# google/forma

Hardware: AMD Instinct MI355X
Metric: frames/sec (sorted+painted, device-resident) + Mpixel-segments/sec (higher is better)
Workload: dtype u64 segments / f64+f32 rasterizer / f32 painter; 1 GPU; paris-like-30k-4k (labelled stand-in: paris-30k.svg is not in the reference checkout); layers=30000, pixel_segments=13757174, frames_in_flight=3

## Files before the change

forma_amd/_lib.py:

```python
from __future__ import annotations

import ctypes as C
import os
import subprocess

_HERE = os.path.dirname(os.path.abspath(__file__))
CSRC = os.path.join(_HERE, "csrc")
SO_PATH = os.environ.get("FORMA_HIP_LIB") or os.path.join(CSRC, "libforma_hip.so")

NONE = 0xFFFFFFFF

ERRORS = {0: "FORMA_OK", -1: "FORMA_E_ARG", -2: "FORMA_E_HIP", -3: "FORMA_E_NO_DEVICE", -4: "FORMA_E_CAPACITY",
          -5: "FORMA_E_STATE", -6: "FORMA_E_INTERNAL", -7: "FORMA_E_COMM"}


class FormaError(RuntimeError):
    def __init__(self, code, msg=""):
        self.code = code
        super().__init__(f"{ERRORS.get(code, code)}: {msg}")


class GeomT(C.Structure):
    _fields_ = [("order", C.c_uint32), ("flags", C.c_uint32), ("xf", C.c_float * 6)]

# ... 18 lines not shown

class ContextInfoT(C.Structure):
    _fields_ = [("n_devices", C.c_uint32), ("frames_in_flight", C.c_uint32), ("transport", C.c_uint32), ("layout", C.c_uint32),
                ("devices", C.c_int32 * 8)]


class KernelTimeT(C.Structure):
    _fields_ = [("name", C.c_char * 48), ("start_us", C.c_float), ("us", C.c_float), ("stage", C.c_uint32), ("reserved", C.c_uint32)]


class SortPlanT(C.Structure):
    _fields_ = [("n_passes", C.c_uint32), ("biased", C.c_uint32), ("shift", C.c_uint32 * 12), ("mask", C.c_uint32 * 12), ("bias", C.c_uint32 * 12)]


class FlattenTablesT(C.Structure):
    _fields_ = [("point_commands", C.c_void_p), ("point_indices", C.c_void_p), ("quad_indices", C.c_void_p), ("n_points", C.c_size_t),
                ("qx", C.c_void_p), ("qy", C.c_void_p), ("qw", C.c_void_p), ("x0", C.c_void_p), ("dx_recip", C.c_void_p),
                ("k0", C.c_void_p), ("dk", C.c_void_p), ("curvatures_recip", C.c_void_p), ("partial_spline", C.c_void_p),
                ("partial_curv", C.c_void_p), ("n_quads", C.c_size_t), ("sp0x", C.c_void_p), ("sp0y", C.c_void_p),
                ("sp2x", C.c_void_p), ("sp2y", C.c_void_p), ("n_splines", C.c_size_t)]


class AffineRangeT(C.Structure):
    _fields_ = [("first", C.c_uint64), ("count", C.c_uint64), ("m", C.c_float * 6)]


class KeepRangeT(C.Structure):
    _fields_ = [("first", C.c_uint64), ("count", C.c_uint64)]


class CountersT(C.Structure):
    _fields_ = [("geometry_points", C.c_uint64), ("geometry_uploads", C.c_uint64), ("geometry_appends", C.c_uint64),
                ("geometry_retains", C.c_uint64), ("geometry_bytes_h2d", C.c_uint64), ("geometry_bytes_d2h", C.c_uint64),
                ("frames", C.c_uint64), ("frames_learned", C.c_uint64), ("frames_rerun", C.c_uint64)]

    def as_dict(self):
        return {k: int(getattr(self, k)) for k, _ in self._fields_}


_vp, _sz, _u32, _i = C.c_void_p, C.c_size_t, C.c_uint32, C.c_int
SYMBOLS = {
    "forma_hip_create": (_i, [C.POINTER(_vp), _i]),
    "forma_hip_create_multi": (_i, [C.POINTER(_vp), C.POINTER(_i), _i]),
    "forma_hip_destroy": (None, [_vp]),
    "forma_hip_last_error": (C.c_char_p, [_vp]),
    "forma_hip_version": (C.c_char_p, []),
    "forma_hip_set_geometry": (_i, [_vp, _vp, _vp, _vp, _sz]),
    "forma_hip_set_geoms": (_i, [_vp, _vp, _sz]),
    "forma_hip_set_styles": (_i, [_vp, _vp, _sz, _vp, _sz, _vp]),
    "forma_hip_set_images": (_i, [_vp, _vp, _sz, _vp, _sz]),
    "forma_hip_flatten": (_i, [_vp, _vp, _vp, _vp]),
    "forma_hip_geometry_append": (_i, [_vp, _vp, _vp, _vp, _sz]),
    "forma_hip_geometry_retain": (_i, [_vp, _vp, _sz, _vp, _sz]),
    "forma_hip_read_geometry": (_i, [_vp, _vp, _vp, _vp, _sz, _vp]),
    "forma_hip_counters": (_i, [_vp, _vp]),
    "forma_hip_prepare_lines": (_i, [_vp, _u32, _u32] + [_vp] * 10),
    "forma_hip_rasterize": (_i, [_vp, _sz] + [_vp] * 10 + [_vp, _sz, _vp]),
    "forma_hip_sort": (_i, [_vp, _vp, _sz, _i]),
    "forma_hip_paint": (_i, [_vp, _vp, _sz, _vp, _u32, _u32, _sz, _vp, _vp, _vp]),
    "forma_hip_render": (_i, [_vp, _vp, _u32, _u32, _sz, _vp, _vp, _vp, _i, _vp]),
    "forma_hip_render_enqueue": (_i, [_vp, _vp, _u32, _u32, _sz, _vp, _vp, _vp]),
    "forma_hip_render_device": (_i, [_vp, _vp, _u32, _u32, _u32, _sz, _vp, _vp, _vp, _i, _vp, _vp]),
    "forma_hip_register_buffer": (_i, [_vp, _vp, _sz]),
    "forma_hip_unregister_buffer": (_i, [_vp, _vp]),
    "forma_hip_cache_clear": (_i, [_vp, _i]),
    "forma_hip_set_frames_in_flight": (_i, [_vp, _i]),
    "forma_hip_multi_layout": (_i, [_vp, _i]),
# ... 48 lines not shown
```

forma_amd/csrc/api.cpp:

```cpp
#include <new>

#include "ctx.h"

#ifndef FORMA_ARCH
#define FORMA_ARCH "gfx950"
#endif

thread_local KernelTimer* g_ktimer = nullptr;
static inline float* kt_us(forma_hip_ctx* c) { return c->kt_dur_us; }

int fd_fail(forma_hip_ctx* c, int code, const char* what, hipError_t e) {
    if (c) snprintf(c->err, sizeof c->err, "%s%s%s", what, e != hipSuccess ? ": " : "", e != hipSuccess ? hipGetErrorString(e) : "");
    return code;
}

namespace {

inline int fail(forma_hip_ctx* c, int code, const char* what, hipError_t e = hipSuccess) { return fd_fail(c, code, what, e); }
void share_scene(forma_hip_ctx* o);
void invalidate_counts(forma_hip_ctx* o);
inline forma_hip_ctx* last_slot(forma_hip_ctx* ctx) { return ctx->last ? ctx->last : ctx; }
#define HIPCHECK(expr)                                                        \
    do {                                                                      \
        hipError_t _e = (expr);                                               \
// ... 102 lines not shown
    ctx->n_lines = n_lines;
    ctx->n_seg = 0; ctx->n_compact = 0; ctx->have_unsorted = true; ctx->live44 = 0; ctx->layer_sorted = true;
    ctx->speculated = false; ctx->ras_hist_on = false; ctx->ras_fused = false;
    ctx->pz = forma_hip_ctx::PreZero();
    int rc = reset_info(ctx);
    if (rc) return rc;
    if (n_lines == 0) return FORMA_OK;
    const LineSource S = geometry_source(ctx, width, height);
    if ((rc = run_line_table(ctx, S, n_lines, timing, bound_n, zero))) return rc;
    if (zero && cleared) ctx->pz = *cleared;
    FrameInfo* dinfo = ctx->info.as<FrameInfo>();
    DevCount nc_seg, nc_cmp;
    if (bound_n) {
        nc_seg = DevCount{&dinfo->n_segments, bound_n};
        nc_cmp = DevCount{&dinfo->n_compact, (uint32_t)n_lines};
    } else {
        const size_t N = ctx->n_seg;
        if (N == 0) return FORMA_OK;
        if (N >= (1ull << 30)) return fail(ctx, FORMA_E_CAPACITY, "more than 2^30-1 pixel segments on one device");
        nc_seg = DevCount{nullptr, (uint32_t)N};
        nc_cmp = DevCount{nullptr, (uint32_t)ctx->n_compact};
    }
    HIPCHECK(ctx->seg_u.ensure(((size_t)nc_seg.bound + SEG_PAD) * 8));
    HIPCHECK(ctx->ras_masks.ensure(((size_t)nc_seg.bound / RAS_TILE + 2) * 32));
    RasHist RH;
    memset(&RH, 0, sizeof RH);
    if (hist_too && bound_n && ctx->pred_valid && ctx->pz.sort_p && ctx->pz.sort_p == ctx->sort_counters.p && !ctx->dbg.no_ras_hist) {
        ctx->ras_plan = frame_sort_plan(ctx, ctx->pred_live44, ctx->pred_layer_sorted, ctx->digit_bits, true, nullptr);
        RH = make_ras_hist(ctx->ras_plan, ctx->sort_counters.as<uint32_t>());
        ctx->ras_hist_on = RH.hist != nullptr;
        if (RH.hist && ctx->pz.slice_p && ctx->pz.slice_p == ctx->slice_buf.p && ctx->pz.slice_words >= slice_tab_words(bound_n) &&
            fuse_plan_ok(ctx, ctx->ras_plan)) {
            const SliceSrc SS = make_slice_src(ctx->slice_buf.as<uint32_t>(), bound_n);
            RH.slice_tab = SS.tab; RH.tab_stride = SS.tab_stride;
            ctx->ras_fused = true;
        }
        {
            const SortPlan plain = make_segment_sort_plan(ctx->pred_live44, ctx->pred_layer_sorted, ctx->digit_bits, nullptr, nullptr);
            const SortPlan lay = ctx->pred_layer_sorted ? SortPlan{} : make_sort_plan((ctx->pred_live44 & 0x1FFFFFull) << 20, 20, 41, ctx->digit_bits);
            bool biased = false;
            for (int p = 0; p < ctx->ras_plan.n_passes; p++) biased |= ctx->ras_plan.fmask[p] != 0u;
            RH.track_range = (biased || plain.n_passes > (ctx->pred_layer_sorted ? 0 : lay.n_passes) + 2) ? 1u : 0u;
        }
    }
    stage_begin(ctx, ST_RASTER, timing);
    launch_rasterize(ctx->stream, S, nc_cmp, nc_seg, ctx->cl_idx.as<uint32_t>(), ctx->cl_start.as<uint32_t>(),
                     ctx->block_first.as<uint32_t>(), ctx->seg_u.as<uint64_t>(), dinfo, (int)ctx->band_row0,
                     (int)ctx->band_row1, ctx->ras_masks.as<uint32_t>(), bound_n == 0, &RH);
    ctx->pending_masks = bound_n ? PendingMasks{ctx->ras_masks.as<uint32_t>(), 0u, ctx->ras_hist_on ? 1u : 0u} : PendingMasks{nullptr, 0u, 0u};
    ctx->seg_u_fused = ctx->ras_fused; ctx->fused_w = width; ctx->fused_h = height;
    stage_end(ctx, ST_RASTER, timing);
    HIPCHECK(hipGetLastError());
    ctx->speculated = (speculate || bound_n) && ctx->pred_valid;
    if (ctx->speculated) {
        ctx->live44 = ctx->pred_live44; ctx->layer_sorted = ctx->pred_layer_sorted;
        return FORMA_OK;
    }
    return finish_rasterize(ctx);
}

static uint32_t sort_workgroups(const forma_hip_ctx* ctx, size_t n_keys) {
    if (ctx->dbg.sort_cus >= 0) return (uint32_t)ctx->dbg.sort_cus;
    const forma_hip_ctx* o = ctx->owner ? ctx->owner : ctx;
    const size_t slots = o->slots.size();
    if (ctx->frame_has_dst) return 0u;
    return slots == 3 || (slots == 2 && n_keys >= ((size_t)1 << 22)) ? o->n_cus / 2u : 0u;
}
// ... 622 lines not shown
            if (ctx->h_stage) (void)hipHostFree(ctx->h_stage);
            ctx->h_stage = nullptr; ctx->h_stage_cap = 0;
            HIPCHECK(hipHostMalloc((void**)&ctx->h_stage, bytes, hipHostMallocDefault));
            ctx->h_stage_cap = bytes;
        }
        HIPCHECK(hipMemcpy2DAsync(ctx->h_stage + py0 * pitch + px0 * 4, pitch, ctx->cur_image + py0 * pitch + px0 * 4, pitch,
                                  (px1 - px0) * 4, py1 - py0, hipMemcpyDeviceToHost, ctx->stream));
        HIPCHECK(hipStreamSynchronize(ctx->stream));
        for (uint32_t ty = ty0; ty < ty1; ty++)
            for (uint32_t tx = tx0; tx < tx1; tx++) {
                if (!ctx->h_written[(size_t)ty * tiles_w + tx]) continue;
                const size_t x0 = (size_t)tx * 16, x1 = std::min<size_t>(x0 + 16, a.width);
                const size_t y0 = (size_t)ty * 16, y1 = std::min<size_t>(y0 + 16, a.height);
                for (size_t y = y0; y < y1; y++) memcpy(dst + y * stride + x0 * 4, ctx->h_stage + y * pitch + x0 * 4, (x1 - x0) * 4);
            }
    }
    stage_end(ctx, ST_D2H, timing);
    return FORMA_OK;
}

int finish_frame(forma_hip_ctx* ctx, forma_timings_t* t, bool have_info = false) {
    if (!have_info) {
        HIPCHECK(hipMemcpyAsync(ctx->h_info, ctx->info.p, sizeof(FrameInfo), hipMemcpyDeviceToHost, ctx->stream));
        HIPCHECK(hipStreamSynchronize(ctx->stream));
    }
    ctx->pred_no_deep = !(ctx->h_info->error & 16u);
    if (ctx->h_info->error & 16u) ctx->cull_on = true;
    if (!ctx->h_info->plan_bad) {
        const uint32_t* r = ctx->h_info->tile_range;
        ctx->pred_range = KeyRange{~r[0], r[1], ~r[2], r[3], true};
    }
    if (!ctx->h_info->plan_bad) ctx->pred_row_spans = ctx->h_info->n_spans / ctx->cur_rows_painted;
    if (!ctx->h_info->plan_bad && ctx->h_info->n_slices) ctx->pred_slice_len = std::max(ctx->h_info->n_segments / ctx->h_info->n_slices, 1u);
    if (!ctx->h_info->plan_bad) { ctx->pred_max_slice = ctx->h_info->max_slice_runs; ctx->pred_slice_n = ctx->cur_slices; ctx->pred_slice_small = ctx->cur_small; ctx->pred_slice_half = ctx->cur_half; }
    if ((ctx->h_info->error & ~24u) == 1u)
        return fail(ctx, FORMA_E_ARG, "a geometry entry names an order that has no style (forma_hip_set_styles: offset FORMA_NONE or beyond the table)");
    if (ctx->h_info->error & ~24u) return fail(ctx, FORMA_E_INTERNAL, "device-side invariant violated");
    if (!t) return FORMA_OK;
    memset(t, 0, sizeof *t);
    float* dstv[ST_COUNT] = {&t->prepare_us, &t->rasterize_us, &t->sort_us, &t->carry_us, &t->paint_us, &t->d2h_us, &t->exchange_us};
    float pass = 0; int np = 0;
    KernelTimer& kt = ctx->kt;
    for (int i = 0; i < kt.n; i++) {
        float ms = 0;
        kt_us(ctx)[i] = 0.0f;
        if (hipEventElapsedTime(&ms, kt.e0[i], kt.e1[i]) != hipSuccess) continue;
        kt_us(ctx)[i] = ms * 1000.0f;
        if (kt.stage[i] >= 0 && kt.stage[i] < ST_COUNT) *dstv[kt.stage[i]] += ms * 1000.0f;
        if (strstr(kt.name[i], "k_onesweep")) { pass += ms * 1000.0f; np++; }
    }
    if (kt.n) {
        float ms = 0;
        if (hipEventElapsedTime(&ms, kt.e0[0], kt.e1[kt.n - 1]) == hipSuccess) t->total_us = ms * 1000.0f;
        for (int i = 0; i < kt.n; i++) {
            ms = 0;
            ctx->kt_start_us[i] = hipEventElapsedTime(&ms, kt.e0[0], kt.e0[i]) == hipSuccess ? ms * 1000.0f : 0.0f;
        }
    }
    ctx->kt_n_done = kt.n;
    if (ctx->stage_used[ST_D2H]) {
        float ms = 0;
        if (hipEventElapsedTime(&ms, ctx->ev0[ST_D2H], ctx->ev1[ST_D2H]) == hipSuccess) t->d2h_us = ms * 1000.0f;
    }
    t->sort_pass_us = np ? pass / np : 0.0f;
    t->n_lines = (uint32_t)ctx->n_lines; t->n_segments = (uint32_t)ctx->n_seg; t->n_sort_passes = (uint32_t)ctx->n_passes;
    t->n_runs = ctx->last_runs ? ctx->last_runs : ctx->h_info->n_runs; t->n_tile_entries = ctx->h_info->n_spans;
// ... 1480 lines not shown
```

forma_amd/csrc/common.h:

```cpp
#pragma once
#include <hip/hip_runtime.h>
#include <hip/hip_ext.h>
#include <stdint.h>
#include <stddef.h>

#include "../../include/forma_hip.h"

#define SEG_KEY_SHIFT 20
#define SEG_KEY_BITS  44

#if defined(__HIPCC__)
#define FD __device__ __forceinline__
#else
#define FD inline
#endif

FD int      seg_tile_y(uint64_t v) { return (int)(v >> 53) - 1; }
FD int      seg_tile_x(uint64_t v) { return (int)((v >> 41) & 0xFFFu) - 1; }
FD uint32_t seg_layer(uint64_t v) { return (uint32_t)(v >> 20) & 0x1FFFFFu; }
FD int      seg_lx(uint64_t v) { return (int)(v >> 16) & 0xF; }
FD int      seg_ly(uint64_t v) { return (int)(v >> 12) & 0xF; }
FD int      seg_dam(uint64_t v) { return (int)(v >> 6) & 0x3F; }
FD int      seg_cover(uint64_t v) { return ((int)(v & 0x3F) ^ 0x20) - 0x20; }
FD uint64_t seg_key(uint64_t v) { return v >> SEG_KEY_SHIFT; }
FD uint32_t seg_tile_key(uint64_t v) { return (uint32_t)(v >> 41); }

struct FrameInfo {
    uint32_t n_segments;
    uint32_t key_or;
    uint32_t key_or_hi;
    uint32_t key_and;
    uint32_t key_and_hi;
    uint32_t seg_begin;
    uint32_t seg_end;
    uint32_t n_runs;
    uint32_t n_spans;
    uint32_t n_entries;
    uint32_t layer_unsorted;
    uint32_t error;
    uint32_t n_compact;
    uint32_t plan_bad;
    uint32_t max_row_runs;
    uint32_t exchange_overflow;
    uint32_t max_slice_runs;
    uint32_t tile_range[4];
    uint32_t n_heavy;
    uint32_t cost_sum, cost_n;
    uint32_t n_slices;
};

struct TileRecord {
    uint32_t cover[4];
    uint32_t seg_start;
    uint32_t seg_count;
    uint32_t layer;
    uint32_t tile;
};

struct PaintParams {
    uint32_t width, height, tiles_w, tiles_h;
    uint32_t crop_x0, crop_x1, crop_y0, crop_y1;
    uint32_t channels;
    float    clear[4];
    uint32_t stride_px;
    uint32_t scene_has_clips;
    uint32_t scene_simple;
    uint32_t n_orders;
    uint32_t n_words;
    uint32_t clear_unchanged;
    uint32_t n_slices;
    uint32_t n_groups;
    uint32_t cull;
    const uint32_t* order_cnt_in;  const uint32_t* order_list_in;  const uint8_t* order_flag_in;
    uint32_t*       order_cnt_out; uint32_t*       order_list_out; uint8_t*       order_flag_out;
    uint32_t        order_hcap, order_thr;
    const uint32_t* row_base; const uint32_t* row_cnt;
};
#define PAINT_RUN_END(P, ty, n_runs) ((P).row_base ? (P).row_base[ty] + (P).row_cnt[ty] : (n_runs))

#ifndef SPAN_GROUP_SHIFT
#define SPAN_GROUP_SHIFT 4
// ... 56 lines not shown
            hipLaunchKernelGGL(kern, grid, block, shm, s, __VA_ARGS__);                                     \
    } while (0)

void launch_prepare_lines(hipStream_t s, const float* x, const float* y, const uint32_t* line_slot, uint32_t n_lines,
                          const forma_geom_t* geoms, uint32_t n_geoms, float width, float height, float band_lo,
                          float band_hi, uint32_t* orders, float* x0, float* y0, float* dx, float* dy, float* a,
                          float* b, float* c, float* d, uint32_t* lengths);
size_t scan_tmp_words(size_t n);
void launch_inclusive_scan_u32(hipStream_t s, uint32_t* data, size_t n, uint32_t* tmp, uint32_t* d_total);
void launch_exclusive_scan_u32(hipStream_t s, uint32_t* data, size_t n, uint32_t* tmp, uint32_t* d_total);
void launch_scan_small_u32(hipStream_t s, uint32_t* data, DevCount n, uint32_t per, uint32_t* d_total);

#define RAS_TILE 2048u
struct PendingMasks { const uint32_t* rec; uint32_t n_fixed; uint32_t has_range; };
struct LineSource {
    const float* x; const float* y; const uint32_t* line_slot; const forma_geom_t* geoms; uint32_t n_geoms;
    float width, height, band_lo, band_hi;
    const uint32_t* sums;
    const uint32_t* orders; const float *x0, *y0, *dx, *dy, *a, *b, *c, *d;
};
size_t prepare_scratch_words(size_t n_lines);
struct ZeroJobs;
void launch_prepare_compact(hipStream_t s, const LineSource& src, uint32_t n_lines, uint32_t* cl_idx, uint32_t* cl_start,
                            uint32_t* block_first, uint32_t bf_cap, uint32_t* scratch, FrameInfo* info,
                            const ZeroJobs* zero );
void launch_line_lengths(hipStream_t s, const LineSource& src, uint32_t n_lines, uint32_t* lens, uint32_t* scratch );
void launch_block_first(hipStream_t s, const uint32_t* cl_start, uint32_t n_compact, uint32_t n_segments,
                        uint32_t* block_first);
#define HS_COPIES  16
#define SORT_BINS  512
#define RH_MAX_PASSES 3
struct RasHist { uint32_t* hist; uint32_t n_passes; uint32_t shift[RH_MAX_PASSES], mask[RH_MAX_PASSES], bias[RH_MAX_PASSES], fmask[RH_MAX_PASSES];
                 uint32_t track_range;
                 uint32_t* slice_tab; uint32_t tab_stride;  };
void launch_rasterize(hipStream_t s, const LineSource& src, DevCount n_compact, DevCount n_segments,
                      const uint32_t* cl_idx, const uint32_t* cl_start, const uint32_t* block_first, uint64_t* out,
                      FrameInfo* info, int band_row0, int band_row1, uint32_t* wg_masks ,
                      bool reduce_now ,
                      const RasHist* hist = nullptr);
void launch_flatten(hipStream_t s, const forma_flatten_tables_t* dev_tables, float* out_x, float* out_y);
struct GeomAppend {
    uint32_t base;
    uint32_t n_affines;
    const uint32_t* affines;
    const uint32_t* slot_in;
    float* x; float* y; uint32_t* slot;
};
void launch_flatten_store(hipStream_t s, const forma_flatten_tables_t* dev_tables, const GeomAppend& A);
constexpr uint32_t GR_THREADS = 256, GR_CHUNK = GR_THREADS * 4;
struct GeomRetain {
    const uint32_t* ranges;
    uint32_t n_keep;
    const uint32_t* remap;
    uint32_t n_slots;
    uint32_t n_out;
    const float* x; const float* y; const uint32_t* slot;
    float* out_x; float* out_y; uint32_t* out_slot;
    uint32_t* flag;
};
void launch_geom_retain(hipStream_t s, const GeomRetain& R);

#define SORT_MAX_PASSES 12
struct SortPlan {
    int      n_passes;
    int      shift[SORT_MAX_PASSES];
    uint32_t mask[SORT_MAX_PASSES];
    uint32_t bias[SORT_MAX_PASSES];
// ... 166 lines not shown
```

forma_amd/csrc/debug.h:

```cpp
#pragma once
#include <cstdlib>
#include <cstring>
#include <algorithm>

struct ForMaDebug {
    bool sync = false, global_runsort = false, xgather = false, no_small_carry = false, span_groups = false, no_span_groups = false;
    bool no_packed_copy = false, no_simple_paint = false, force_simple_paint = false, trim_debug = false, force_exchange = false;
    bool xchg_copy = false, no_prezero = false, no_bias = false, no_ras_hist = false, no_cull = false, force_cull = false, no_order = false;
    int carry_slices = 0, digit_bits = 0, poison = -1, poison_frame = -1, strip_tiles = -1, carry_half = 1, paint_quad = 1, order_thr = -1, sort_cus = -1, runs_chain = -1, multi_layout = 0, carry_covl = 1, runs_blk = -1, blk_round = 256, tail_poll = 1, paint_split = 1, split_first = 25, fuse_digit = 1;
};

inline ForMaDebug forma_debug_parse() {
    ForMaDebug d;
    const char* e = getenv("FORMA_HIP_DEBUG");
    if (!e) return d;
    char buf[512];
    strncpy(buf, e, sizeof buf - 1); buf[sizeof buf - 1] = 0;
    char* save = nullptr;
    for (char* tok = strtok_r(buf, ",; ", &save); tok; tok = strtok_r(nullptr, ",; ", &save)) {
        char* val = strchr(tok, '=');
        if (val) *val++ = 0;
        const long v = val ? strtol(val, nullptr, 0) : 0;
#define FD_FLAG(name) if (!strcmp(tok, #name)) { d.name = true; continue; }
        FD_FLAG(sync) FD_FLAG(global_runsort) FD_FLAG(xgather) FD_FLAG(no_small_carry) FD_FLAG(span_groups) FD_FLAG(no_span_groups)
        FD_FLAG(no_cull) FD_FLAG(force_cull) FD_FLAG(no_order) FD_FLAG(no_prezero) FD_FLAG(no_bias) FD_FLAG(no_ras_hist) FD_FLAG(no_packed_copy) FD_FLAG(no_simple_paint) FD_FLAG(force_simple_paint) FD_FLAG(trim_debug) FD_FLAG(force_exchange)
#undef FD_FLAG
        if (!strcmp(tok, "xchg")) { d.xchg_copy = val && !strcmp(val, "copy"); continue; }
        if (!strcmp(tok, "multi_layout")) { d.multi_layout = val && !strcmp(val, "exchange") ? 1 : (val && !strcmp(val, "bands") ? 2 : 0); continue; }
        if (!strcmp(tok, "carry_slices")) { d.carry_slices = (int)v; continue; }
        if (!strcmp(tok, "digit_bits")) { d.digit_bits = (int)v; continue; }
        if (!strcmp(tok, "carry_half")) { d.carry_half = (int)std::max(v, 0L); continue; }
        if (!strcmp(tok, "carry_covl")) { d.carry_covl = (int)std::max(v, 0L); continue; }
        if (!strcmp(tok, "sort_cus")) { d.sort_cus = (int)std::max(v, 0L); continue; }
        if (!strcmp(tok, "order_thr")) { d.order_thr = (int)std::max(v, 0L); continue; }
        if (!strcmp(tok, "paint_quad")) { d.paint_quad = (int)std::max(v, 0L); continue; }
        if (!strcmp(tok, "runs_chain")) { d.runs_chain = (int)std::max(v, 0L); continue; }
        if (!strcmp(tok, "runs_blk")) { d.runs_blk = (int)std::max(v, 0L); continue; }
        if (!strcmp(tok, "blk_round")) { d.blk_round = (int)std::min(std::max(v, 1L), 256L); continue; }
        if (!strcmp(tok, "paint_split")) { d.paint_split = (int)std::min(std::max(v, 0L), 8L); continue; }
        if (!strcmp(tok, "split_first")) { d.split_first = (int)std::min(std::max(v, 1L), 99L); continue; }
        if (!strcmp(tok, "fuse_digit")) { d.fuse_digit = (int)std::min(std::max(v, 0L), 2L); continue; }
        if (!strcmp(tok, "tail_poll")) { d.tail_poll = (int)std::max(v, 0L); continue; }
        if (!strcmp(tok, "strip_tiles")) { d.strip_tiles = (int)std::max(v, 0L); continue; }
        if (!strcmp(tok, "poison")) { d.poison = (int)(v & 0xFF); continue; }
        if (!strcmp(tok, "poison_frame")) { d.poison_frame = (int)(v & 0xFF); continue; }
    }
    return d;
}
```

forma_amd/csrc/lines.hip:

```cpp
#include "common.h"
#include "lookback.h"
#include "radix_rank.h"
#include <string.h>
#ifdef RAS_PROF
__device__ unsigned long long g_ras_prof[64][8];
#define RP_STAMP(i) do { const unsigned long long _t = __builtin_readcyclecounter(); if (threadIdx.x == 0) atomicAdd(&g_ras_prof[blockIdx.x & 63][i], _t - rp_t); rp_t = __builtin_readcyclecounter(); } while (0)
extern "C" int forma_hip_debug_ras_prof(unsigned long long* out8, int reset) {
    static unsigned long long h[64][8];
    if (reset) { for (int c = 0; c < 64; c++) for (int i = 0; i < 8; i++) h[c][i] = 0; return (int)hipMemcpyToSymbol(HIP_SYMBOL(g_ras_prof), h, sizeof h); }
    int rc = (int)hipMemcpyFromSymbol(h, HIP_SYMBOL(g_ras_prof), sizeof h);
    for (int i = 0; i < 8; i++) { out8[i] = 0; for (int c = 0; c < 64; c++) out8[i] += h[c][i]; }
    return rc;
}
#else
#define RP_STAMP(i) do { } while (0)
#endif

#define WAVE 64

__device__ __forceinline__ uint32_t wave_inclusive_scan(uint32_t v) {
    const int lane = threadIdx.x & 63;
#pragma unroll
    for (int d = 1; d < 64; d <<= 1) {
        uint32_t t = __shfl_up(v, d, 64);
// ... 465 lines not shown
    int cover = (int)(int8_t)(y1s - y0s);
    int ty1 = (int)(int16_t)(tile_y + 1), tx1 = (int)(int16_t)(tile_x + 1);
    uint64_t v = (uint64_t)(ty1 > 0 ? ty1 : 0) & 0x7FFull;
    v = (v << 12) | ((uint64_t)(tx1 > 0 ? tx1 : 0) & 0xFFFull);
    v = (v << 21) | ((uint64_t)order & 0x1FFFFFull);
    v = (v << 4) | lx;
    v = (v << 4) | ly;
    v = (v << 6) | (dam & 0x3Fu);
    v = (v << 6) | ((uint32_t)cover & 0x3Fu);
    return v;
}

__device__ __forceinline__ LineP load_line(const LineSource& S, uint32_t li) {
    if (S.sums) {
        LineP L;
        L.order = S.orders[li]; L.x0 = S.x0[li]; L.y0 = S.y0[li]; L.dx = S.dx[li]; L.dy = S.dy[li];
        L.a = S.a[li]; L.b = S.b[li]; L.c = S.c[li]; L.d = S.d[li]; L.len = 1;
        return L;
    }
    return line_params(S.x, S.y, S.line_slot, li, S.geoms, S.n_geoms, S.width, S.height, S.band_lo, S.band_hi);
}

#ifndef RAS_OCC
#define RAS_OCC 6
#endif
struct RasWindow {
    double aab[RAS_WIN], bab[RAS_WIN], cdab[RAS_WIN], cdb[RAS_WIN];
    float x0[RAS_WIN], y0[RAS_WIN], dx[RAS_WIN], dy[RAS_WIN], a[RAS_WIN], b[RAS_WIN], c[RAS_WIN], d[RAS_WIN];
    uint32_t start[RAS_WIN + 1], order[RAS_WIN];
    int ioff[RAS_WIN];
};
union RasLds { RasWindow w; uint64_t stg[RAS_TILE]; };
static_assert(sizeof(uint64_t) * RAS_TILE <= sizeof(RasWindow), "the partition staging lives in the line window");

__device__ __forceinline__ void ras_partition(const uint64_t (&vout)[RAS_PER_THREAD], uint64_t* __restrict__ out, const RasHist& RH,
                                              uint64_t* stg, uint16_t* wc , uint32_t* wsum ,
                                              uint32_t k0, uint32_t k1) {
    constexpr int WAVES = RAS_THREADS / 64, PER_WAVE = 64 * RAS_PER_THREAD;
    static_assert(WAVES * 256 * 2 <= SORT_BINS * 4, "the wave counters live in lh's first row");
    static_assert(RAS_THREADS == 256, "one digit per thread");
    const int tid = threadIdx.x, lane = tid & 63, w = tid >> 6;
    const uint32_t sh = RH.shift[0], mk = RH.mask[0], bs = RH.bias[0];
    const uint32_t nloc = k1 - k0;
#pragma unroll
    for (int q = 0; q < RAS_PER_THREAD; q += 2)
        *reinterpret_cast<ulonglong2*>(&stg[tid * RAS_PER_THREAD + q]) = make_ulonglong2(vout[q], vout[q + 1]);
    __syncthreads();
    uint64_t kk[RAS_PER_THREAD];
    uint32_t rk[RAS_PER_THREAD / 2];
    uint32_t* wcw = reinterpret_cast<uint32_t*>(wc) + w * 128;
#pragma unroll
    for (int j = 0; j < RAS_PER_THREAD; j++) {
        const uint32_t i = w * PER_WAVE + j * 64 + lane;
        kk[j] = stg[i];
        const uint32_t dg = i < nloc ? (((uint32_t)(kk[j] >> sh) - bs) & mk) : mk;
        uint32_t mlo, mhi;
        match_any<8>(dg, mlo, mhi);
        const uint32_t below = lanes_below(mlo, mhi), cnt = (uint32_t)__popc(mlo) + (uint32_t)__popc(mhi);
        const uint32_t hs = (dg & 1u) * 16u;
        if (below == 0) atomicAdd(&wcw[dg >> 1], cnt << hs);
        __builtin_amdgcn_fence(__ATOMIC_RELEASE, "wavefront");
        const uint32_t r = ((wcw[dg >> 1] >> hs) & 0xFFFFu) - cnt + below;
        if (j & 1) rk[j >> 1] |= r << 16; else rk[j >> 1] = r;
    }
    __syncthreads();
    {
        const uint32_t d = (uint32_t)tid;
        uint32_t c[WAVES], tot = 0;
#pragma unroll
        for (int q = 0; q < WAVES; q++) { c[q] = wc[q * 256 + d]; tot += c[q]; }
        uint32_t incl = tot;
#pragma unroll
        for (int o = 1; o < 64; o <<= 1) { const uint32_t v = __shfl_up(incl, o, 64); if (lane >= o) incl += v; }
        if (lane == 63) wsum[w] = incl;
        __syncthreads();
        uint32_t off = incl - tot;
        for (int q = 0; q < w; q++) off += wsum[q];
        uint32_t acc = off;
#pragma unroll
        for (int q = 0; q < WAVES; q++) { wc[q * 256 + d] = (uint16_t)acc; acc += c[q]; }
        if (d == mk) tot -= RAS_TILE - nloc;
        if (tot) {
            RH.slice_tab[(size_t)d * RH.tab_stride + blockIdx.x] = (off << 12) | tot;
            uint32_t* mine = RH.hist + (size_t)(blockIdx.x % HS_COPIES) * (SORT_MAX_PASSES * SORT_BINS);
            atomicAdd(&mine[d], tot);
            atomicAdd(&mine[SLICE_NZ_ROW * SORT_BINS + d], 1u);
        }
    }
    __syncthreads();
#pragma unroll
    for (int j = 0; j < RAS_PER_THREAD; j++) {
        const uint32_t i = w * PER_WAVE + j * 64 + lane;
        const uint32_t dg = i < nloc ? (((uint32_t)(kk[j] >> sh) - bs) & mk) : mk;
        stg[wc[w * 256 + dg] + ((rk[j >> 1] >> ((j & 1) * 16)) & 0xFFFFu)] = kk[j];
    }
    __syncthreads();
#pragma unroll
    for (int q = 0; q < RAS_PER_THREAD; q += 2) {
        const uint32_t i = (uint32_t)q * RAS_THREADS + 2u * tid;
        if (i + 1 < nloc) *reinterpret_cast<ulonglong2*>(out + k0 + i) = *reinterpret_cast<const ulonglong2*>(&stg[i]);
        else if (i < nloc) out[k0 + i] = stg[i];
    }
}

template <bool HIST, bool FUSE = false>
__global__ __launch_bounds__(RAS_THREADS, RAS_OCC) void k_rasterize(LineSource S, DevCount nc_compact, DevCount nc_segments,
                                                           const uint32_t* __restrict__ cl_idx,
                                                           const uint32_t* __restrict__ cl_start,
                                                           const uint32_t* __restrict__ block_first,
                                                           uint64_t* __restrict__ out, FrameInfo* __restrict__ info,
                                                           int band_row0, int band_row1, uint32_t* __restrict__ wg_masks,
                                                           RasHist RH) {
    __shared__ uint32_t lh[HIST ? RH_MAX_PASSES * SORT_BINS : 1];
    __shared__ RasLds lw;
    uint32_t (&w_start)[RAS_WIN + 1] = lw.w.start;
    uint32_t (&w_order)[RAS_WIN] = lw.w.order;
    float (&w_x0)[RAS_WIN] = lw.w.x0; float (&w_y0)[RAS_WIN] = lw.w.y0; float (&w_dx)[RAS_WIN] = lw.w.dx; float (&w_dy)[RAS_WIN] = lw.w.dy;
    float (&w_a)[RAS_WIN] = lw.w.a; float (&w_b)[RAS_WIN] = lw.w.b; float (&w_c)[RAS_WIN] = lw.w.c; float (&w_d)[RAS_WIN] = lw.w.d;
    double (&w_aab)[RAS_WIN] = lw.w.aab; double (&w_bab)[RAS_WIN] = lw.w.bab; double (&w_cdab)[RAS_WIN] = lw.w.cdab; double (&w_cdb)[RAS_WIN] = lw.w.cdb;
    int (&w_ioff)[RAS_WIN] = lw.w.ioff;
    __shared__ uint32_t red[HIST ? (FUSE ? 8 : 7) : 5][RAS_THREADS / 64];
    const int tid = threadIdx.x;
    const uint32_t n_segments = dev_count(nc_segments), n_compact = dev_count(nc_compact);
    const uint32_t bf_lo = block_first[blockIdx.x], bf_hi = block_first[blockIdx.x + 1];
    const uint32_t nblocks = (n_segments + RAS_TILE - 1) / RAS_TILE;
    const uint32_t k0 = blockIdx.x * RAS_TILE;
    if (k0 >= n_segments) return;
    const uint32_t k1 = min(k0 + RAS_TILE, n_segments);
#ifdef RAS_PROF
    unsigned long long rp_t = __builtin_readcyclecounter();
    if (tid == 0) atomicAdd(&g_ras_prof[blockIdx.x & 63][7], 1ull);
#endif
    const uint32_t lo = bf_lo;
    const uint32_t hi = blockIdx.x + 1 < nblocks ? bf_hi : n_compact - 1;
    uint32_t k_or = 0, k_or_hi = 0, k_and = 0xFFFFFFFFu, k_and_hi = 0xFFFFFFFFu, unsorted = 0;
// ... 108 lines not shown
                }
                if (nv == RAS_PER_THREAD) atomicAdd(&h[d[RAS_PER_THREAD - 1]], c);
            }
        }
    }
    if constexpr (!FUSE) {
#pragma unroll
    for (int q = 0; q < RAS_PER_THREAD; q += 2) {
        const uint32_t k = kt + q;
        if (k + 1 < k1) *reinterpret_cast<ulonglong2*>(out + k) = make_ulonglong2(vout[q], vout[q + 1]);
        else if (k < k1) out[k] = vout[q];
    }
    }
#pragma unroll
    for (int d = 32; d >= 1; d >>= 1) {
        k_or |= __shfl_xor(k_or, d, 64); k_or_hi |= __shfl_xor(k_or_hi, d, 64);
        k_and &= __shfl_xor(k_and, d, 64); k_and_hi &= __shfl_xor(k_and_hi, d, 64);
        unsorted |= __shfl_xor(unsorted, d, 64);
    }
    if (HIST && RH.track_range) {
#pragma unroll
        for (int d = 32; d >= 1; d >>= 1) {
            min_x = min(min_x, (uint32_t)__shfl_xor(min_x, d, 64)); max_x = max(max_x, (uint32_t)__shfl_xor(max_x, d, 64));
            min_y = min(min_y, (uint32_t)__shfl_xor(min_y, d, 64)); max_y = max(max_y, (uint32_t)__shfl_xor(max_y, d, 64));
        }
    }
    const int w = tid >> 6;
    __syncthreads();
    if ((tid & 63) == 0) {
        red[0][w] = k_or; red[1][w] = k_or_hi; red[2][w] = k_and; red[3][w] = k_and_hi; red[4][w] = unsorted;
        if (HIST) { red[5][w] = min_x | (max_x << 16); red[6][w] = min_y | (max_y << 16); }
    }
    __syncthreads();
    if constexpr (FUSE) ras_partition(vout, out, RH, lw.stg, reinterpret_cast<uint16_t*>(lh), red[7], k0, k1);
    if (HIST) {
        uint32_t* mine = RH.hist + (size_t)(blockIdx.x % HS_COPIES) * (SORT_MAX_PASSES * SORT_BINS);
        for (uint32_t i = tid + (FUSE ? SORT_BINS : 0u); i < RH.n_passes * SORT_BINS; i += RAS_THREADS) {
            const uint32_t v = lh[i];
            if (v) atomicAdd(&mine[i], v);
        }
    }
    if (tid == 0) {
        uint32_t o = 0, oh = 0, a = 0xFFFFFFFFu, ah = 0xFFFFFFFFu, u = 0;
        for (int i = 0; i < RAS_THREADS / 64; i++) { o |= red[0][i]; oh |= red[1][i]; a &= red[2][i]; ah &= red[3][i]; u |= red[4][i]; }
        if (HIST) {
            uint32_t lo_x = 0xFFFFu, hi_x = 0, lo_y = 0xFFFFu, hi_y = 0;
            for (int i = 0; i < RAS_THREADS / 64; i++) {
                lo_x = min(lo_x, red[5][i] & 0xFFFFu); hi_x = max(hi_x, red[5][i] >> 16);
                lo_y = min(lo_y, red[6][i] & 0xFFFFu); hi_y = max(hi_y, red[6][i] >> 16);
            }
            uint32_t* mr = wg_masks + (size_t)blockIdx.x * 8;
            mr[5] = lo_x | (hi_x << 16); mr[6] = lo_y | (hi_y << 16);
            for (uint32_t p = 0; p < RH.n_passes; p++) {
                if (!RH.fmask[p]) continue;
                const bool is_x = RH.shift[p] == 41;
                const uint32_t lo_v = is_x ? lo_x : lo_y, hi_v = is_x ? hi_x : hi_y;
                if (lo_v < RH.bias[p] || hi_v - RH.bias[p] > RH.mask[p]) info->plan_bad = 1u;
            }
        }
        uint32_t* m = wg_masks + (size_t)blockIdx.x * 8;
        m[0] = o; m[1] = oh; m[2] = a; m[3] = ah; m[4] = u;
    }
    RP_STAMP(3);
}

__global__ __launch_bounds__(1024) void k_reduce_masks(const uint32_t* __restrict__ wg_masks, DevCount nc_segments,
                                                       FrameInfo* __restrict__ info) {
// ... 181 lines not shown
```

include/forma_hip.h:

```cpp
#ifndef FORMA_HIP_H
#define FORMA_HIP_H

#include <stddef.h>
#include <stdint.h>

#ifdef __cplusplus
extern "C" {
#endif

#define FORMA_MAX_WIDTH   65536u
#define FORMA_MAX_HEIGHT  32768u
#define FORMA_LAYER_LIMIT 0x1FFFFFu
#define FORMA_TILE        16u
#define FORMA_NONE        0xFFFFFFFFu

#define FORMA_OK             0
#define FORMA_E_ARG         -1
#define FORMA_E_HIP         -2
#define FORMA_E_NO_DEVICE   -3
#define FORMA_E_CAPACITY    -4
#define FORMA_E_STATE       -5
#define FORMA_E_INTERNAL    -6
#define FORMA_E_COMM        -7

// ... 65 lines not shown

typedef struct forma_flatten_tables_t {
    const uint32_t* point_commands;
    const uint32_t* point_indices;
    const uint32_t* quad_indices;
    size_t          n_points;
    const float* qx; const float* qy; const float* qw;
    const float* x0; const float* dx_recip; const float* k0; const float* dk;
    const float* curvatures_recip;
    const uint32_t* partial_spline;
    const float*    partial_curv;
    size_t          n_quads;
    const float* sp0x; const float* sp0y; const float* sp2x; const float* sp2y;
    size_t       n_splines;
} forma_flatten_tables_t;
int forma_hip_flatten(forma_hip_ctx* ctx, const forma_flatten_tables_t* t,
                      float* out_x, float* out_y);

typedef struct forma_affine_range_t { uint64_t first, count; float m[6]; } forma_affine_range_t;
typedef struct forma_keep_range_t   { uint64_t first, count; } forma_keep_range_t;
int forma_hip_geometry_append(forma_hip_ctx* ctx, const forma_flatten_tables_t* t, const uint32_t* line_slot,
                              const forma_affine_range_t* affines, size_t n_affines);
int forma_hip_geometry_retain(forma_hip_ctx* ctx, const forma_keep_range_t* keep, size_t n_keep,
                              const uint32_t* slot_remap, size_t n_slots);
int forma_hip_read_geometry(forma_hip_ctx* ctx, float* x, float* y, uint32_t* line_slot,
                            size_t capacity_points, size_t* out_points);
typedef struct forma_counters_t {
    uint64_t geometry_points;
    uint64_t geometry_uploads, geometry_appends, geometry_retains;
    uint64_t geometry_bytes_h2d, geometry_bytes_d2h;
    uint64_t frames;
    uint64_t frames_learned;
    uint64_t frames_rerun;
} forma_counters_t;
int forma_hip_counters(forma_hip_ctx* ctx, forma_counters_t* out);

int forma_hip_prepare_lines(forma_hip_ctx* ctx, uint32_t width, uint32_t height,
                            uint32_t* orders, float* x0, float* y0, float* dx, float* dy,
                            float* a, float* b, float* c, float* d, uint32_t* lengths);
int forma_hip_rasterize(forma_hip_ctx* ctx, size_t n_lines,
                        const uint32_t* orders, const float* x0, const float* y0,
                        const float* dx, const float* dy, const float* a, const float* b,
                        const float* c, const float* d, const uint32_t* lengths,
                        uint64_t* out_segments, size_t capacity, size_t* out_n);
int forma_hip_sort(forma_hip_ctx* ctx, uint64_t* segments, size_t n, int digit_bits);
int forma_hip_paint(forma_hip_ctx* ctx, const uint64_t* sorted_segments, size_t n,
                    uint8_t* dst, uint32_t width, uint32_t height, size_t stride_bytes,
                    const uint8_t channels[4], const float clear_color[4],
                    const forma_rect_t* crop_or_null);

int forma_hip_render(forma_hip_ctx* ctx, uint8_t* dst, uint32_t width, uint32_t height,
                     size_t stride_bytes, const uint8_t channels[4],
                     const float clear_color[4], const forma_rect_t* crop_or_null,
                     int cache_id, forma_timings_t* timings);
int forma_hip_render_enqueue(forma_hip_ctx* ctx, uint8_t* dst, uint32_t width, uint32_t height,
                             size_t stride_bytes, const uint8_t channels[4],
                             const float clear_color[4], const forma_rect_t* crop_or_null);
#define FORMA_FORMAT_SRGB8      0u
#define FORMA_FORMAT_LINEAR_F16 1u
int forma_hip_render_device(forma_hip_ctx* ctx, void* dst_device, uint32_t format,
                            uint32_t width, uint32_t height, size_t stride_bytes,
                            const uint8_t channels[4], const float clear_color[4],
                            const forma_rect_t* crop_or_null, int cache_id,
                            void* wait_stream , forma_timings_t* timings);
int forma_hip_register_buffer(forma_hip_ctx* ctx, void* ptr, size_t bytes);
int forma_hip_unregister_buffer(forma_hip_ctx* ctx, void* ptr);
// ... 68 lines not shown
```

rust/forma_hip/ffi.rs:

```rust

#![allow(non_camel_case_types, dead_code)]

use std::os::raw::{c_char, c_int, c_void};

pub const FORMA_NONE: u32 = 0xFFFF_FFFF;

pub const FORMA_OK: c_int = 0;
pub const FORMA_E_ARG: c_int = -1;
pub const FORMA_E_HIP: c_int = -2;
pub const FORMA_E_NO_DEVICE: c_int = -3;
pub const FORMA_E_CAPACITY: c_int = -4;
pub const FORMA_E_STATE: c_int = -5;
pub const FORMA_E_INTERNAL: c_int = -6;
pub const FORMA_E_COMM: c_int = -7;

pub const FORMA_GEOM_HAS_XF: u32 = 1;

pub const FORMA_FORMAT_SRGB8: u32 = 0;
pub const FORMA_FORMAT_LINEAR_F16: u32 = 1;

pub const FORMA_FILL_SOLID: u32 = 0;
pub const FORMA_FILL_LINEAR: u32 = 1;
pub const FORMA_FILL_RADIAL: u32 = 2;
pub const FORMA_FILL_TEXTURE: u32 = 3;
// ... 102 lines not shown
    pub frames_in_flight: u32,
    pub transport: u32,
    pub layout: u32,
    pub devices: [i32; FORMA_MAX_DEVICES],
}

#[repr(C)]
#[derive(Clone, Copy, Debug, Default)]
pub struct forma_affine_range_t {
    pub first: u64,
    pub count: u64,
    pub m: [f32; 6],
}

#[repr(C)]
#[derive(Clone, Copy, Debug, Default)]
pub struct forma_keep_range_t {
    pub first: u64,
    pub count: u64,
}

#[repr(C)]
#[derive(Clone, Copy, Debug, Default)]
pub struct forma_counters_t {
    pub geometry_points: u64,
    pub geometry_uploads: u64,
    pub geometry_appends: u64,
    pub geometry_retains: u64,
    pub geometry_bytes_h2d: u64,
    pub geometry_bytes_d2h: u64,
    pub frames: u64,
    pub frames_learned: u64,
    pub frames_rerun: u64,
}

#[repr(C)]
#[derive(Clone, Copy, Debug)]
pub struct forma_kernel_time_t {
    pub name: [c_char; 48],
    pub start_us: f32,
    pub us: f32,
    pub stage: u32,
    pub reserved: u32,
}

pub const FORMA_SORT_MAX_PASSES: usize = 12;

#[repr(C)]
#[derive(Clone, Copy, Debug, Default)]
pub struct forma_sort_plan_t {
    pub n_passes: u32,
    pub biased: u32,
    pub shift: [u32; FORMA_SORT_MAX_PASSES],
    pub mask: [u32; FORMA_SORT_MAX_PASSES],
    pub bias: [u32; FORMA_SORT_MAX_PASSES],
}

#[link(name = "forma_hip")]
extern "C" {
    pub fn forma_hip_create(out: *mut *mut forma_hip_ctx, device: c_int) -> c_int;
    pub fn forma_hip_create_multi(out: *mut *mut forma_hip_ctx, devices: *const c_int, n: c_int) -> c_int;
    pub fn forma_hip_destroy(ctx: *mut forma_hip_ctx);
    pub fn forma_hip_last_error(ctx: *const forma_hip_ctx) -> *const c_char;
    pub fn forma_hip_version() -> *const c_char;

    pub fn forma_hip_set_geometry(
// ... 222 lines not shown
```

Baseline: 3083 frames/s.

## Partition fused rasterizer output by digit runs instead of per-element ranking

```diff
diff --git a/forma_amd/_lib.py b/forma_amd/_lib.py
--- a/forma_amd/_lib.py
+++ b/forma_amd/_lib.py
@@ -74,7 +74,8 @@
 class CountersT(C.Structure):
     _fields_ = [("geometry_points", C.c_uint64), ("geometry_uploads", C.c_uint64), ("geometry_appends", C.c_uint64),
                 ("geometry_retains", C.c_uint64), ("geometry_bytes_h2d", C.c_uint64), ("geometry_bytes_d2h", C.c_uint64),
-                ("frames", C.c_uint64), ("frames_learned", C.c_uint64), ("frames_rerun", C.c_uint64)]
+                ("frames", C.c_uint64), ("frames_learned", C.c_uint64), ("frames_rerun", C.c_uint64),
+                ("fused_blocks", C.c_uint64), ("fused_blocks_fallback", C.c_uint64)]
 
     def as_dict(self):
         return {k: int(getattr(self, k)) for k, _ in self._fields_}
diff --git a/forma_amd/csrc/api.cpp b/forma_amd/csrc/api.cpp
--- a/forma_amd/csrc/api.cpp
+++ b/forma_amd/csrc/api.cpp
@@ -158,7 +158,7 @@
         if (RH.hist && ctx->pz.slice_p && ctx->pz.slice_p == ctx->slice_buf.p && ctx->pz.slice_words >= slice_tab_words(bound_n) &&
             fuse_plan_ok(ctx, ctx->ras_plan)) {
             const SliceSrc SS = make_slice_src(ctx->slice_buf.as<uint32_t>(), bound_n);
-            RH.slice_tab = SS.tab; RH.tab_stride = SS.tab_stride;
+            RH.slice_tab = SS.tab; RH.tab_stride = SS.tab_stride; RH.part_mode = (uint32_t)ctx->dbg.part_runs;
             ctx->ras_fused = true;
         }
         {
@@ -847,6 +847,10 @@
     }
     if (!ctx->h_info->plan_bad) ctx->pred_row_spans = ctx->h_info->n_spans / ctx->cur_rows_painted;
     if (!ctx->h_info->plan_bad && ctx->h_info->n_slices) ctx->pred_slice_len = std::max(ctx->h_info->n_segments / ctx->h_info->n_slices, 1u);
+    if (!ctx->h_info->plan_bad && ctx->h_info->n_slices) {
+        forma_counters_t& c = (ctx->owner ? ctx->owner : ctx)->cnt;
+        c.fused_blocks += (ctx->h_info->n_segments + RAS_TILE - 1) / RAS_TILE; c.fused_blocks_fallback += ctx->h_info->n_part_fallback;
+    }
     if (!ctx->h_info->plan_bad) { ctx->pred_max_slice = ctx->h_info->max_slice_runs; ctx->pred_slice_n = ctx->cur_slices; ctx->pred_slice_small = ctx->cur_small; ctx->pred_slice_half = ctx->cur_half; }
     if ((ctx->h_info->error & ~24u) == 1u)
         return fail(ctx, FORMA_E_ARG, "a geometry entry names an order that has no style (forma_hip_set_styles: offset FORMA_NONE or beyond the table)");
diff --git a/forma_amd/csrc/common.h b/forma_amd/csrc/common.h
--- a/forma_amd/csrc/common.h
+++ b/forma_amd/csrc/common.h
@@ -47,6 +47,7 @@
     uint32_t n_heavy;
     uint32_t cost_sum, cost_n;
     uint32_t n_slices;
+    uint32_t n_part_fallback;
 };
 
 struct TileRecord {
@@ -169,7 +170,8 @@
 #define RH_MAX_PASSES 3
 struct RasHist { uint32_t* hist; uint32_t n_passes; uint32_t shift[RH_MAX_PASSES], mask[RH_MAX_PASSES], bias[RH_MAX_PASSES], fmask[RH_MAX_PASSES];
                  uint32_t track_range;
-                 uint32_t* slice_tab; uint32_t tab_stride;  };
+                 uint32_t* slice_tab; uint32_t tab_stride;
+                 uint32_t part_mode;  };
 void launch_rasterize(hipStream_t s, const LineSource& src, DevCount n_compact, DevCount n_segments,
                       const uint32_t* cl_idx, const uint32_t* cl_start, const uint32_t* block_first, uint64_t* out,
                       FrameInfo* info, int band_row0, int band_row1, uint32_t* wg_masks ,
diff --git a/forma_amd/csrc/debug.h b/forma_amd/csrc/debug.h
--- a/forma_amd/csrc/debug.h
+++ b/forma_amd/csrc/debug.h
@@ -7,7 +7,7 @@
     bool sync = false, global_runsort = false, xgather = false, no_small_carry = false, span_groups = false, no_span_groups = false;
     bool no_packed_copy = false, no_simple_paint = false, force_simple_paint = false, trim_debug = false, force_exchange = false;
     bool xchg_copy = false, no_prezero = false, no_bias = false, no_ras_hist = false, no_cull = false, force_cull = false, no_order = false;
-    int carry_slices = 0, digit_bits = 0, poison = -1, poison_frame = -1, strip_tiles = -1, carry_half = 1, paint_quad = 1, order_thr = -1, sort_cus = -1, runs_chain = -1, multi_layout = 0, carry_covl = 1, runs_blk = -1, blk_round = 256, tail_poll = 1, paint_split = 1, split_first = 25, fuse_digit = 1;
+    int carry_slices = 0, digit_bits = 0, poison = -1, poison_frame = -1, strip_tiles = -1, carry_half = 1, paint_quad = 1, order_thr = -1, sort_cus = -1, runs_chain = -1, multi_layout = 0, carry_covl = 1, runs_blk = -1, blk_round = 256, tail_poll = 1, paint_split = 1, split_first = 25, fuse_digit = 1, part_runs = 1;
 };
 
 inline ForMaDebug forma_debug_parse() {
@@ -40,6 +40,7 @@
         if (!strcmp(tok, "paint_split")) { d.paint_split = (int)std::min(std::max(v, 0L), 8L); continue; }
         if (!strcmp(tok, "split_first")) { d.split_first = (int)std::min(std::max(v, 1L), 99L); continue; }
         if (!strcmp(tok, "fuse_digit")) { d.fuse_digit = (int)std::min(std::max(v, 0L), 2L); continue; }
+        if (!strcmp(tok, "part_runs")) { d.part_runs = (int)std::min(std::max(v, 0L), 2L); continue; }
         if (!strcmp(tok, "tail_poll")) { d.tail_poll = (int)std::max(v, 0L); continue; }
         if (!strcmp(tok, "strip_tiles")) { d.strip_tiles = (int)std::max(v, 0L); continue; }
         if (!strcmp(tok, "poison")) { d.poison = (int)(v & 0xFF); continue; }
diff --git a/forma_amd/csrc/lines.hip b/forma_amd/csrc/lines.hip
--- a/forma_amd/csrc/lines.hip
+++ b/forma_amd/csrc/lines.hip
@@ -521,38 +521,128 @@
 };
 union RasLds { RasWindow w; uint64_t stg[RAS_TILE]; };
 static_assert(sizeof(uint64_t) * RAS_TILE <= sizeof(RasWindow), "the partition staging lives in the line window");
-
+constexpr int RAS_WAVES = RAS_THREADS / 64;
+constexpr int RAS_RUN_CAP = ((int)((sizeof(RasLds) - sizeof(uint64_t) * RAS_TILE) / 4) - RAS_WAVES) / RAS_WAVES;
+static_assert(RAS_RUN_CAP >= 64, "a wavefront's run table holds at least one row of runs");
+
+__device__ __forceinline__ uint32_t ras_stg_slot(uint32_t p) { return p ^ (((p >> 4) & 7u) << 1); }
+#ifdef RAS_PROF
+#define RP_ARG , unsigned long long& rp_t
+#define RP_PASS , rp_t
+#else
+#define RP_ARG
+#define RP_PASS
+#endif
 __device__ __forceinline__ void ras_partition(const uint64_t (&vout)[RAS_PER_THREAD], uint64_t* __restrict__ out, const RasHist& RH,
-                                              uint64_t* stg, uint16_t* wc , uint32_t* wsum ,
-                                              uint32_t k0, uint32_t k1) {
-    constexpr int WAVES = RAS_THREADS / 64, PER_WAVE = 64 * RAS_PER_THREAD;
+                                              FrameInfo* __restrict__ info, uint64_t* stg, uint32_t* tabs ,
+                                              uint16_t* wc , uint32_t* wsum ,
+                                              uint32_t k0, uint32_t k1 RP_ARG) {
+    constexpr int WAVES = RAS_WAVES, PER_WAVE = 64 * RAS_PER_THREAD;
     static_assert(WAVES * 256 * 2 <= SORT_BINS * 4, "the wave counters live in lh's first row");
     static_assert(RAS_THREADS == 256, "one digit per thread");
     const int tid = threadIdx.x, lane = tid & 63, w = tid >> 6;
     const uint32_t sh = RH.shift[0], mk = RH.mask[0], bs = RH.bias[0];
     const uint32_t nloc = k1 - k0;
-#pragma unroll
-    for (int q = 0; q < RAS_PER_THREAD; q += 2)
-        *reinterpret_cast<ulonglong2*>(&stg[tid * RAS_PER_THREAD + q]) = make_ulonglong2(vout[q], vout[q + 1]);
+    uint32_t* wcw = reinterpret_cast<uint32_t*>(wc) + w * 128;
+    uint32_t* tab = tabs + w * RAS_RUN_CAP;
+    uint32_t* nrw = tabs + WAVES * RAS_RUN_CAP;
+    const uint32_t lpos = (uint32_t)lane * RAS_PER_THREAD;
+    uint32_t dg[RAS_PER_THREAD];
+    if (sh >= 32) {
+#pragma unroll
+        for (int q = 0; q < RAS_PER_THREAD; q++) dg[q] = (((uint32_t)(vout[q] >> 32) >> (sh - 32)) - bs) & mk;
+    } else {
+#pragma unroll
+        for (int q = 0; q < RAS_PER_THREAD; q++) dg[q] = ((uint32_t)(vout[q] >> sh) - bs) & mk;
+    }
+    if ((uint32_t)(tid + 1) * RAS_PER_THREAD > nloc) {
+#pragma unroll
+        for (int q = 0; q < RAS_PER_THREAD; q++) if ((uint32_t)tid * RAS_PER_THREAD + q >= nloc) dg[q] = mk;
+    }
+    bool brk[RAS_PER_THREAD];
+    uint32_t excl = 0, nr = 0;
+    {
+        const uint32_t pv = (uint32_t)__shfl_up((int)dg[RAS_PER_THREAD - 1], 1, 64);
+        brk[0] = lane == 0 || pv != dg[0];
+#pragma unroll
+        for (int q = 1; q < RAS_PER_THREAD; q++) brk[q] = dg[q] != dg[q - 1];
+#pragma unroll
+        for (int q = 0; q < RAS_PER_THREAD; q++) {
+            const uint64_t bal = __ballot(brk[q]);
+            excl = __builtin_amdgcn_mbcnt_hi((uint32_t)(bal >> 32), __builtin_amdgcn_mbcnt_lo((uint32_t)bal, excl));
+            nr += (uint32_t)__popcll(bal);
+        }
+    }
+    nr = (uint32_t)__builtin_amdgcn_readfirstlane((int)nr);
+    const bool fits = nr <= (uint32_t)RAS_RUN_CAP && RH.part_mode != 0u;
+    if (lane == 0) nrw[w] = fits ? 0u : 1u;
+    if (fits) {
+        uint32_t run = excl - 1u;
+#pragma unroll
+        for (int q = 0; q < RAS_PER_THREAD; q++) {
+            run += brk[q] ? 1u : 0u;
+            if (brk[q]) tab[run] = dg[q] | ((lpos + (uint32_t)q) << 8);
+        }
+        __builtin_amdgcn_fence(__ATOMIC_RELEASE, "wavefront");
+        __builtin_amdgcn_wave_barrier();
+        const uint32_t lt_lo = lane < 32 ? (1u << lane) - 1u : ~0u, lt_hi = lane < 32 ? 0u : (1u << (lane - 32)) - 1u;
+        for (uint32_t r0 = 0; r0 < nr; r0 += 64) {
+            const uint32_t r = r0 + (uint32_t)lane;
+            const bool valid = r < nr;
+            const uint32_t e = tab[min(r, (uint32_t)RAS_RUN_CAP - 1u)], en = tab[min(r + 1u, (uint32_t)RAS_RUN_CAP - 1u)];
+            const uint32_t start = e >> 8, end = r + 1u < nr ? en >> 8 : (uint32_t)PER_WAVE;
+            const uint32_t len = valid ? end - start : 0u, d = valid ? e & 0xFFu : 0u;
+            uint32_t mlo, mhi;
+            match_any<8>(d, mlo, mhi);
+            uint64_t mb = ((uint64_t)(mhi & lt_hi) << 32) | (mlo & lt_lo);
+            uint32_t below = 0;
+            while (__any(mb != 0ull)) {
+                const bool more = mb != 0ull;
+                const uint32_t v = (uint32_t)__shfl((int)len, more ? __builtin_ctzll(mb) : lane, 64);
+                below += more ? v : 0u;
+                mb &= mb - 1ull;
+            }
+            const bool last = lanes_below(mlo, mhi) + 1u == (uint32_t)__popc(mlo) + (uint32_t)__popc(mhi);
+            const uint32_t hs = (d & 1u) * 16u;
+            const uint32_t old = (wcw[d >> 1] >> hs) & 0xFFFFu;
+            __builtin_amdgcn_fence(__ATOMIC_RELEASE, "wavefront");
+            if (last) atomicAdd(&wcw[d >> 1], (below + len) << hs);
+            if (valid) tab[r] = d | ((old + below + (uint32_t)PER_WAVE - start) << 8);
+            __builtin_amdgcn_fence(__ATOMIC_RELEASE, "wavefront");
+        }
+    }
+    RP_STAMP(4);
     __syncthreads();
+    const bool fb = (nrw[0] | nrw[1] | nrw[2] | nrw[3]) != 0u;
+    static_assert(WAVES == 4, "four run counts");
     uint64_t kk[RAS_PER_THREAD];
     uint32_t rk[RAS_PER_THREAD / 2];
-    uint32_t* wcw = reinterpret_cast<uint32_t*>(wc) + w * 128;
-#pragma unroll
-    for (int j = 0; j < RAS_PER_THREAD; j++) {
-        const uint32_t i = w * PER_WAVE + j * 64 + lane;
-        kk[j] = stg[i];
-        const uint32_t dg = i < nloc ? (((uint32_t)(kk[j] >> sh) - bs) & mk) : mk;
-        uint32_t mlo, mhi;
-        match_any<8>(dg, mlo, mhi);
-        const uint32_t below = lanes_below(mlo, mhi), cnt = (uint32_t)__popc(mlo) + (uint32_t)__popc(mhi);
-        const uint32_t hs = (dg & 1u) * 16u;
-        if (below == 0) atomicAdd(&wcw[dg >> 1], cnt << hs);
-        __builtin_amdgcn_fence(__ATOMIC_RELEASE, "wavefront");
-        const uint32_t r = ((wcw[dg >> 1] >> hs) & 0xFFFFu) - cnt + below;
-        if (j & 1) rk[j >> 1] |= r << 16; else rk[j >> 1] = r;
-    }
-    __syncthreads();
+    if (fb) {
+        if (tid == 0) {
+            if (RH.part_mode == 2u) info->plan_bad = 1u;
+            atomicAdd(&info->n_part_fallback, 1u);
+        }
+        for (int i = tid; i < WAVES * 128; i += RAS_THREADS) reinterpret_cast<uint32_t*>(wc)[i] = 0;
+#pragma unroll
+        for (int q = 0; q < RAS_PER_THREAD; q += 2)
+            *reinterpret_cast<ulonglong2*>(&stg[tid * RAS_PER_THREAD + q]) = make_ulonglong2(vout[q], vout[q + 1]);
+        __syncthreads();
+#pragma unroll
+        for (int j = 0; j < RAS_PER_THREAD; j++) {
+            const uint32_t i = w * PER_WAVE + j * 64 + lane;
+            kk[j] = stg[i];
+            const uint32_t d = i < nloc ? (((uint32_t)(kk[j] >> sh) - bs) & mk) : mk;
+            uint32_t mlo, mhi;
+            match_any<8>(d, mlo, mhi);
+            const uint32_t below = lanes_below(mlo, mhi), cnt = (uint32_t)__popc(mlo) + (uint32_t)__popc(mhi);
+            const uint32_t hs = (d & 1u) * 16u;
+            if (below == 0) atomicAdd(&wcw[d >> 1], cnt << hs);
+            __builtin_amdgcn_fence(__ATOMIC_RELEASE, "wavefront");
+            const uint32_t r = ((wcw[d >> 1] >> hs) & 0xFFFFu) - cnt + below;
+            if (j & 1) rk[j >> 1] |= r << 16; else rk[j >> 1] = r;
+        }
+        __syncthreads();
+    }
     {
         const uint32_t d = (uint32_t)tid;
         uint32_t c[WAVES], tot = 0;
@@ -576,20 +666,37 @@
             atomicAdd(&mine[SLICE_NZ_ROW * SORT_BINS + d], 1u);
         }
     }
+    RP_STAMP(5);
     __syncthreads();
-#pragma unroll
-    for (int j = 0; j < RAS_PER_THREAD; j++) {
-        const uint32_t i = w * PER_WAVE + j * 64 + lane;
-        const uint32_t dg = i < nloc ? (((uint32_t)(kk[j] >> sh) - bs) & mk) : mk;
-        stg[wc[w * 256 + dg] + ((rk[j >> 1] >> ((j & 1) * 16)) & 0xFFFFu)] = kk[j];
+    if (fb) {
+#pragma unroll
+        for (int j = 0; j < RAS_PER_THREAD; j++) {
+            const uint32_t i = w * PER_WAVE + j * 64 + lane;
+            const uint32_t d = i < nloc ? (((uint32_t)(kk[j] >> sh) - bs) & mk) : mk;
+            stg[ras_stg_slot(wc[w * 256 + d] + ((rk[j >> 1] >> ((j & 1) * 16)) & 0xFFFFu))] = kk[j];
+        }
+    } else {
+        for (uint32_t r0 = 0; r0 < nr; r0 += 64) {
+            const uint32_t r = r0 + (uint32_t)lane;
+            if (r < nr) { const uint32_t e = tab[r]; tab[r] = (uint32_t)wc[w * 256 + (e & 0xFFu)] + (e >> 8) - (uint32_t)PER_WAVE; }
+        }
+        __builtin_amdgcn_fence(__ATOMIC_RELEASE, "wavefront");
+        __builtin_amdgcn_wave_barrier();
+        uint32_t run = excl - 1u;
+#pragma unroll
+        for (int q = 0; q < RAS_PER_THREAD; q++) {
+            run += brk[q] ? 1u : 0u;
+            stg[ras_stg_slot(lpos + (uint32_t)q + tab[run])] = vout[q];
+        }
     }
     __syncthreads();
 #pragma unroll
     for (int q = 0; q < RAS_PER_THREAD; q += 2) {
         const uint32_t i = (uint32_t)q * RAS_THREADS + 2u * tid;
-        if (i + 1 < nloc) *reinterpret_cast<ulonglong2*>(out + k0 + i) = *reinterpret_cast<const ulonglong2*>(&stg[i]);
-        else if (i < nloc) out[k0 + i] = stg[i];
-    }
+        if (i + 1 < nloc) *reinterpret_cast<ulonglong2*>(out + k0 + i) = *reinterpret_cast<const ulonglong2*>(&stg[ras_stg_slot(i)]);
+        else if (i < nloc) out[k0 + i] = stg[ras_stg_slot(i)];
+    }
+    RP_STAMP(6);
 }
 
 template <bool HIST, bool FUSE = false>
@@ -764,7 +871,10 @@
         if (HIST) { red[5][w] = min_x | (max_x << 16); red[6][w] = min_y | (max_y << 16); }
     }
     __syncthreads();
-    if constexpr (FUSE) ras_partition(vout, out, RH, lw.stg, reinterpret_cast<uint16_t*>(lh), red[7], k0, k1);
+    if constexpr (FUSE) {
+        RP_STAMP(3);
+        ras_partition(vout, out, RH, info, lw.stg, reinterpret_cast<uint32_t*>(&lw.stg[RAS_TILE]), reinterpret_cast<uint16_t*>(lh), red[7], k0, k1 RP_PASS);
+    }
     if (HIST) {
         uint32_t* mine = RH.hist + (size_t)(blockIdx.x % HS_COPIES) * (SORT_MAX_PASSES * SORT_BINS);
         for (uint32_t i = tid + (FUSE ? SORT_BINS : 0u); i < RH.n_passes * SORT_BINS; i += RAS_THREADS) {
diff --git a/include/forma_hip.h b/include/forma_hip.h
--- a/include/forma_hip.h
+++ b/include/forma_hip.h
@@ -121,6 +121,8 @@
     uint64_t frames;
     uint64_t frames_learned;
     uint64_t frames_rerun;
+    uint64_t fused_blocks;
+    uint64_t fused_blocks_fallback;
 } forma_counters_t;
 int forma_hip_counters(forma_hip_ctx* ctx, forma_counters_t* out);
 
diff --git a/rust/forma_hip/ffi.rs b/rust/forma_hip/ffi.rs
--- a/rust/forma_hip/ffi.rs
+++ b/rust/forma_hip/ffi.rs
@@ -158,6 +158,8 @@
     pub frames: u64,
     pub frames_learned: u64,
     pub frames_rerun: u64,
+    pub fused_blocks: u64,
+    pub fused_blocks_fallback: u64,
 }
 
 #[repr(C)]
```

Result: slower. 2992 frames/s (-3.0%).
